# gabinsane/multimodal-vae-comparison

Hardware: AMD Instinct MI355X
Metric: training samples/sec, MoPoE CdSprites+ L2 (fwd+bwd+Adam) (higher is better)
Workload: dtype f32; 1 GPU; configs[1]: MoPoE, CdSprites+ L2 shapes, CNN2 image tower + TxtTransformer text tower, n_latents=32, batch=128/GPU, T=32; Adam(amsgrad) lr 1e-4, beta 1, train mode (dropout on); global_batch=128, parallelism=dp1, settle_steps=40

## Files before the change

### include/mmvae_hip.h

```cpp
#ifndef MMVAE_HIP_H
#define MMVAE_HIP_H

#include <stddef.h>
#include <stdint.h>

#ifdef __cplusplus
extern "C" {
#endif

typedef void* mmvae_stream_t;

enum {
  MMVAE_OK = 0,
  MMVAE_ERR_ARG = 1,
  MMVAE_ERR_UNSUPPORTED = 2,
  MMVAE_ERR_LAUNCH = 3,
  MMVAE_ERR_NO_CONVERGENCE = 4
};

enum { MMVAE_ACT_NONE = 0, MMVAE_ACT_SILU = 1, MMVAE_ACT_RELU = 2, MMVAE_ACT_GELU = 3 };
enum {
  MMVAE_EP_NONE = 0,
  MMVAE_EP_RELU = 1,
  MMVAE_EP_MUL_RELU_MASK = 2,
// ... 26 lines not shown
                                 const mmvae_dropout_t* drop, mmvae_stream_t stream);

int mmvae_ffn32_supported(int d_model, int FF);
int mmvae_proj32_ln_fwd(const float* x, const float* w, const float* b, const float* r, const float* gamma, const float* beta,
                        float* y, float* xhat, float* rstd, int M, const mmvae_dropout_t* drop, mmvae_stream_t stream);
int mmvae_ffn32_bwd_parts(int M, int FF);
size_t mmvae_ffn32_bwd_rowlen(int FF);
int mmvae_ffn32_fwd(const float* x, const float* w1, const float* b1, const float* w2, const float* b2, float* y, int M,
                    int FF, const mmvae_dropout_t* drop, mmvae_stream_t stream);
int mmvae_ffn32_bwd(const float* x, const float* dy, const float* w1, const float* b1, const float* w2, float* dx,
                    float* ws, int M, int FF, const mmvae_dropout_t* drop, mmvae_stream_t stream);
size_t mmvae_ffn32_wsplit_bytes(int FF);
size_t mmvae_ffn32_rsplit_bytes(int M);
int mmvae_ffn32_prep_weights(const float* w1, const float* w2, void* wsplit, int FF, mmvae_stream_t stream);
int mmvae_ffn32_prep_weights_many(const float* const* w1, const float* const* w2, void* const* wsplit, int n, int FF,
                                  mmvae_stream_t stream);
int mmvae_ffn32_fwd_b16(const float* x, const void* wsplit, const float* b1, const float* b2, float* y, int M, int FF,
                        const mmvae_dropout_t* drop, mmvae_stream_t stream);
int mmvae_ffn32_fwd_b16_ln(const float* x, const void* wsplit, const float* b1, const float* b2, const float* r,
                           const float* gamma, const float* beta, float* y, float* xhat, float* rstd, int M, int FF,
                           const mmvae_dropout_t* drop, const mmvae_dropout_t* ln_drop, mmvae_stream_t stream);
int mmvae_ffn32_bwd_b16(const float* x, const float* dy, const void* wsplit, const float* b1, float* dx, float* ws,
                        void* rsplit, const float* dx_add, int M, int FF, const mmvae_dropout_t* drop,
                        mmvae_stream_t stream);

int mmvae_version(void);
const char* mmvae_arch(void);


int mmvae_conv2d_k4s2_fwd(const float* x, const float* w, const float* bias, const float* aux, float* y,
                          int B, int Cin, int Cout, int Hin, int in_act, int ep_mode, mmvae_stream_t stream);

int mmvae_conv2d_k4s2_dgrad(const float* dy, const float* w, const float* aux, float* dx,
                            int B, int Cin, int Cout, int Hout, int ep_mode, mmvae_stream_t stream);

int mmvae_conv2d_k4s2_wgrad(const float* dy, const float* x, float* dw, float* db, float* ws,
                            int B, int Cin, int Cout, int Hout, int x_act, int accumulate, mmvae_stream_t stream);

int mmvae_convT2d_k4s2_fwd(const float* x, const float* w, const float* bias, const float* aux, float* y,
                           int B, int Cin, int Cout, int Hin, int in_act, int ep_mode, mmvae_stream_t stream);

int mmvae_convT2d_k4s2_dgrad(const float* dy, const float* w, const float* aux, float* dx,
                             int B, int Cin, int Cout, int Hin, int ep_mode, mmvae_stream_t stream);

int mmvae_convT2d_k4s2_wgrad(const float* x, const float* dy, float* dw, float* db, float* ws,
                             int B, int Cin, int Cout, int Hin, int x_act, int accumulate, mmvae_stream_t stream);

size_t mmvae_conv_wgrad_ws_floats(int B, int Csmall, int Clarge, int Hsmall);

int mmvae_conv2d_k4s2_bwd(const float* dy, const float* x, const float* w, float* dx, float* dw, float* db, float* ws,
                          int B, int Cin, int Cout, int Hout, int x_act, int accumulate, mmvae_stream_t stream);
int mmvae_convT2d_k4s2_bwd(const float* dy, const float* x, const float* w, float* dx, float* dw, float* db, float* ws,
                           int B, int Cin, int Cout, int Hin, int x_act, int accumulate, mmvae_stream_t stream);
int mmvae_convT3_bce_seeded(const float* x, const float* w, const float* bias, const float* target, float* row,
                            float* dlogit, float* part, unsigned* ticket, int B, int in_act, float seed,
                            mmvae_stream_t stream);
int mmvae_convT3_bce_strips(int B);
int mmvae_conv_plan(int split_bf16);

int mmvae_gemm_f32(const float* A, const float* Bm, const float* bias, const float* aux, float* C,
                   float* a_rowsum, float* ws, int M, int N, int K, long sam, long sak, long sbk, long sbn,
                   long ldc, int a_act, int b_act, int ep_mode, int accumulate, int splitk,
                   mmvae_stream_t stream);
size_t mmvae_gemm_ws_floats(int M, int N, int splitk);
int mmvae_gemm_splits(int M, int N, int K, int splitk);
int mmvae_gemm_b16_set(int on);
int mmvae_bias_group_add(float* y, const float* bias, int rows, int C, int G, mmvae_stream_t stream);
size_t mmvae_bias_group_ws_floats(int rows, int C);
int mmvae_bias_group_parts(int rows);
int mmvae_bias_group_grad(const float* dy, float* db, float* ws, int rows, int C, int G, int accumulate,
                          mmvae_stream_t stream);

int mmvae_linear_fwd(const float* x, const float* w, const float* b, float* aux, float* y, int M, int N, int K,
                     long ldx, int x_act, int ep_mode, mmvae_stream_t stream);
int mmvae_linear_bwd_data(const float* dy, const float* w, const float* aux, float* dx, int M, int N, int K,
                          int ep_mode, int accumulate, mmvae_stream_t stream);
int mmvae_linear_bwd_weight(const float* dy, const float* x, float* dw, float* db, float* ws, int M, int N, int K,
                            long ldx, int x_act, int accumulate, mmvae_stream_t stream);
size_t mmvae_linear_bwd_weight_ws_floats(int M, int N, int K);
#define MMVAE_WGRAD_BATCH_MAX 8
typedef struct {
  const float* dy; const float* x; float* dw; float* db; float* ws;
  int M, N, K; long ldx; int x_act, accumulate;
} mmvae_wgrad_job_t;
int mmvae_linear_bwd_weight_batch(const mmvae_wgrad_job_t* jobs, int n_jobs, mmvae_stream_t stream);
typedef struct {
  const float* dy; const float* x; float* ws;
  int M, N, K;
} mmvae_txt_wgrad_job_t;
int mmvae_txt_wgrad(const mmvae_txt_wgrad_job_t* jobs, int n_jobs, mmvae_stream_t stream);
int mmvae_txt_wgrad_splits(int M, int N, int K);
size_t mmvae_txt_wgrad_ws_floats(int M, int N, int K);
int mmvae_txt_wgrad_supported(int M, int N, int K);
int mmvae_linear_bwd(const float* dy, const float* x, const float* w, const float* aux, float* dx, float* dw,
                     float* db, float* ws, int M, int N, int K, long ldx, int x_act, int ep_mode, int accumulate,
                     mmvae_stream_t stream);
size_t mmvae_linear_bwd_ws_floats(int M, int N, int K);

int mmvae_head_softmax_fwd(float* h, int B, int D, mmvae_stream_t stream);
int mmvae_head_softmax_bwd(const float* h, float* dh, int B, int D, mmvae_stream_t stream);

#define MMVAE_MAX_EXPERTS 8
typedef struct {
  const float* mu[MMVAE_MAX_EXPERTS];
  const float* lv[MMVAE_MAX_EXPERTS];
  const float* eps[MMVAE_MAX_EXPERTS];
// ... 605 lines not shown
```

### multimodal_vae_comparison_amd/csrc/conv.hip

```cpp
#include "conv_common.hpp"

#include "conv_gather.inc"
#include "conv_gather_b16.inc"
#include "conv_scatter.inc"
#include "conv_scatter_b16.inc"
#include "conv_wgrad.inc"

constexpr int cmax(int a, int b) { return a > b ? a : b; }

template <typename G, typename W, bool SPEC = false>
__global__ __launch_bounds__(256) void conv2d_bwd_fused_kernel(ConvScatterArgs ad, ConvWgradArgs aw, int n_w, int w_gx) {
  MMVAE_TRACE_STAMP(10 + G::LGH);
  __shared__ __attribute__((aligned(16))) float smem[cmax(G::SMEM, W::SMEM)];
  if ((int)blockIdx.x < n_w) conv_wgrad_body<W, SPEC>(aw, blockIdx.x % w_gx, blockIdx.x / w_gx, w_gx, smem);
  else
    conv_scatter_body<G>(ad, (n_w & 7) ? (int)blockIdx.x - n_w : xcd_contiguous(blockIdx.x - n_w, gridDim.x - n_w), smem);
}
template <typename G, typename W, bool SPEC = false>
__global__ __launch_bounds__(256) void convT_bwd_fused_kernel(ConvGatherArgs ad, ConvWgradArgs aw, int n_w, int w_gx) {
  MMVAE_TRACE_STAMP(14 - G::LGH);
  __shared__ __attribute__((aligned(16))) float smem[cmax(G::SMEM, W::SMEM)];
  if ((int)blockIdx.x < n_w) conv_wgrad_body<W, SPEC>(aw, blockIdx.x % w_gx, blockIdx.x / w_gx, w_gx, smem);
  else
    conv_gather_body<G, G::RWONLY>(ad, (n_w & 7) ? (int)blockIdx.x - n_w : xcd_contiguous(blockIdx.x - n_w, gridDim.x - n_w),
// ... 175 lines not shown
  if (rc) return rc;
  return conv_bwd_reduce(ws, dw, db, B, Cout, Hin, Cout, accumulate, stream);
}

extern "C" int mmvae_conv2d_k4s2_fwd(const float* x, const float* w, const float* bias, const float* aux, float* y,
                                     int B, int Cin, int Cout, int Hin, int in_act, int ep_mode,
                                     mmvae_stream_t stream) {
  MMVAE_CHECK_ARG(x && w && y && B > 0);
  return conv_gather_dispatch(x, w, bias, aux, y, B, Cin, Cout, Hin, in_act, ep_mode, (hipStream_t)stream);
}
extern "C" int mmvae_conv2d_k4s2_dgrad(const float* dy, const float* w, const float* aux, float* dx, int B, int Cin,
                                       int Cout, int Hout, int ep_mode, mmvae_stream_t stream) {
  MMVAE_CHECK_ARG(dy && w && dx && B > 0);
  return conv_scatter_dispatch(dy, w, nullptr, aux, dx, B, Cout, Cin, Hout, MMVAE_ACT_NONE, ep_mode,
                               (hipStream_t)stream);
}
extern "C" int mmvae_conv2d_k4s2_wgrad(const float* dy, const float* x, float* dw, float* db, float* ws, int B,
                                       int Cin, int Cout, int Hout, int x_act, int accumulate,
                                       mmvae_stream_t stream) {
  MMVAE_CHECK_ARG(dy && x && dw && B > 0);
  return conv_wgrad_dispatch(dy, x, dw, db, ws, B, Cout, Cin, Hout, MMVAE_ACT_NONE, x_act, 1, accumulate,
                             (hipStream_t)stream);
}
extern "C" int mmvae_convT2d_k4s2_fwd(const float* x, const float* w, const float* bias, const float* aux, float* y,
                                      int B, int Cin, int Cout, int Hin, int in_act, int ep_mode,
                                      mmvae_stream_t stream) {
  MMVAE_CHECK_ARG(x && w && y && B > 0);
  return conv_scatter_dispatch(x, w, bias, aux, y, B, Cin, Cout, Hin, in_act, ep_mode, (hipStream_t)stream);
}
extern "C" int mmvae_convT3_bce_seeded(const float* x, const float* w, const float* bias, const float* target, float* row,
                                       float* dlogit, float* part, unsigned* ticket, int B, int in_act, float seed,
                                       mmvae_stream_t stream) {
  MMVAE_CHECK_ARG(x && w && target && row && dlogit && B > 0);
  MMVAE_CHECK_ARG(in_act == MMVAE_ACT_NONE || in_act == MMVAE_ACT_RELU || in_act == MMVAE_ACT_SILU);
  MMVAE_CHECK_ARG(convT3_strips(B) == 1 || (part && ticket));
  MMVAE_CHECK_ARG((((uintptr_t)target | (uintptr_t)dlogit) & 15) == 0);
  ConvT3Args t{x, w, bias, dlogit, target, row, part, ticket, B, in_act, MMVAE_EP_SIGMOID_CLAMP, seed};
  convT3_launch<true>(t, (hipStream_t)stream);
  return mmvae_launch_status();
}
extern "C" int mmvae_convT2d_k4s2_dgrad(const float* dy, const float* w, const float* aux, float* dx, int B, int Cin,
                                        int Cout, int Hin, int ep_mode, mmvae_stream_t stream) {
  MMVAE_CHECK_ARG(dy && w && dx && B > 0);
  return conv_gather_dispatch(dy, w, nullptr, aux, dx, B, Cout, Cin, 2 * Hin, MMVAE_ACT_NONE, ep_mode,
                              (hipStream_t)stream);
}
extern "C" int mmvae_convT2d_k4s2_wgrad(const float* x, const float* dy, float* dw, float* db, float* ws, int B,
                                        int Cin, int Cout, int Hin, int x_act, int accumulate,
                                        mmvae_stream_t stream) {
  MMVAE_CHECK_ARG(x && dy && dw && B > 0);
  return conv_wgrad_dispatch(x, dy, dw, db, ws, B, Cin, Cout, Hin, x_act, MMVAE_ACT_NONE, 2, accumulate,
                             (hipStream_t)stream);
}
extern "C" size_t mmvae_conv_wgrad_ws_floats(int B, int Csmall, int Clarge, int Hsmall) {
  return conv_wgrad_ws_floats(B, Csmall, Clarge, Hsmall);
}
extern "C" int mmvae_conv_wgrad_layout(int B, int Csmall, int Clarge, int Hsmall, int* rows, int* rowlen,
                                       int* bias_col) {
  MMVAE_CHECK_ARG(rows && rowlen && bias_col);
  conv_wgrad_layout(B, Csmall, Clarge, Hsmall, rows, rowlen, bias_col);
  return MMVAE_OK;
}

MMVAE_TRACE_SETTER(conv)

extern "C" int mmvae_conv_plan(int split_bf16) {
  const int old = g_conv_split_bf16;
  if (split_bf16 >= 0) g_conv_split_bf16 = split_bf16 ? 1 : 0;
  return old;
}
```

### multimodal_vae_comparison_amd/hipops.py

```python
import ctypes
import os

import torch

_HERE = os.path.dirname(os.path.abspath(__file__))
LIB_PATH = os.path.join(_HERE, "libmmvae_hip.so")
_lib = None

c_p = ctypes.c_void_p
c_i = ctypes.c_int
c_l = ctypes.c_long
c_f = ctypes.c_float
c_u = ctypes.c_uint
c_sz = ctypes.c_size_t
c_d = ctypes.c_double

MAX_EXPERTS = 8

ACT_NONE, ACT_SILU, ACT_RELU, ACT_GELU = 0, 1, 2, 3
EP_NONE, EP_RELU, EP_MUL_RELU_MASK, EP_MUL_SILU_GRAD, EP_GELU, EP_MUL_GELU_GRAD, EP_SIGMOID_CLAMP, EP_SIGMOID, EP_ADD_AUX = range(9)

ERR_ARG, ERR_UNSUPPORTED, ERR_LAUNCH, ERR_NO_CONVERGENCE = 1, 2, 3, 4
_ERR = {ERR_ARG: "invalid argument", ERR_UNSUPPORTED: "unsupported shape", ERR_LAUNCH: "kernel launch failed",
        ERR_NO_CONVERGENCE: "no convergence within the iteration cap"}
# ... 64 lines not shown

class RcStat(ctypes.Structure):
    _fields_ = [("Y", c_p), ("mean", c_p), ("rstd", c_p), ("gamma", c_p), ("pqr", c_p), ("dgamma", c_p), ("dbeta", c_p),
                ("part", c_p), ("counter", c_p), ("acc", c_i), ("eval", c_i)]


class RcGeom(ctypes.Structure):
    _fields_ = [("H", c_i), ("W", c_i), ("Ho", c_i), ("Wo", c_i), ("KW", c_i), ("S", c_i), ("P", c_i)]


class RcFwd(ctypes.Structure):
    _fields_ = [("x", c_p), ("w", c_p), ("xmean", c_p), ("xsc", c_p), ("xbeta", c_p), ("y", c_p), ("ws", c_p),
                ("tile_ticket", c_p), ("M", c_i), ("Cin", c_i), ("Cout", c_i), ("T", c_i), ("pre", c_i), ("g", RcGeom),
                ("gamma", c_p),
                ("beta", c_p), ("run_mean", c_p), ("run_var", c_p), ("mean", c_p), ("rstd", c_p), ("sc", c_p), ("part", c_p),
                ("counter", c_p), ("eps", c_f), ("momentum", c_f), ("eval", c_i)]


class RcDgrad(ctypes.Structure):
    _fields_ = [("G", c_p), ("Y", c_p), ("pqr", c_p), ("w", c_p), ("add", c_p), ("add_tbl", c_p), ("mask", c_i),
                ("mY", c_p), ("mmean", c_p), ("msc", c_p), ("mbeta", c_p), ("out", c_p), ("ws", c_p), ("tile_ticket", c_p),
                ("row_map", c_p), ("M", c_i), ("Min", c_i), ("Cin", c_i), ("Cout", c_i), ("T", c_i), ("nstat", c_i), ("g", RcGeom),
                ("st", RcStat * 2)]


class RcWgrad(ctypes.Structure):
    _fields_ = [("G", c_p), ("Y", c_p), ("pqr", c_p), ("x", c_p), ("xmean", c_p), ("xsc", c_p), ("xbeta", c_p), ("tbl", c_p),
                ("dw", c_p), ("ws", c_p), ("counter", c_p), ("M", c_i), ("Cin", c_i), ("Cout", c_i), ("T", c_i), ("pre", c_i),
                ("accumulate", c_i)]


RC_MAX_JOBS = 8


class RcJob(ctypes.Structure):
    _fields_ = [("kind", c_i), ("f", RcFwd), ("d", RcDgrad), ("w", RcWgrad)]


c_dp = ctypes.POINTER(Dropout)
DROPOUT_SLOTS = 16

SIGNATURES = {
    "mmvae_version": (c_i, []),
    "mmvae_arch": (ctypes.c_char_p, []),
    "mmvae_conv2d_k4s2_fwd": (c_i, [c_p] * 5 + [c_i] * 6 + [c_p]),
    "mmvae_conv2d_k4s2_dgrad": (c_i, [c_p] * 4 + [c_i] * 5 + [c_p]),
    "mmvae_conv2d_k4s2_wgrad": (c_i, [c_p] * 5 + [c_i] * 6 + [c_p]),
    "mmvae_convT2d_k4s2_fwd": (c_i, [c_p] * 5 + [c_i] * 6 + [c_p]),
    "mmvae_convT2d_k4s2_dgrad": (c_i, [c_p] * 4 + [c_i] * 5 + [c_p]),
    "mmvae_convT2d_k4s2_wgrad": (c_i, [c_p] * 5 + [c_i] * 6 + [c_p]),
    "mmvae_conv_wgrad_ws_floats": (c_sz, [c_i] * 4),
    "mmvae_conv2d_k4s2_bwd": (c_i, [c_p] * 7 + [c_i] * 6 + [c_p]),
    "mmvae_convT2d_k4s2_bwd": (c_i, [c_p] * 7 + [c_i] * 6 + [c_p]),
    "mmvae_gemm_f32": (c_i, [c_p] * 7 + [c_i] * 3 + [c_l] * 5 + [c_i] * 5 + [c_p]),
    "mmvae_gemm_ws_floats": (c_sz, [c_i] * 3),
    "mmvae_gemm_splits": (c_i, [c_i] * 4),
    "mmvae_bias_group_add": (c_i, [c_p, c_p, c_i, c_i, c_i, c_p]),
    "mmvae_bias_group_grad": (c_i, [c_p, c_p, c_p, c_i, c_i, c_i, c_i, c_p]),
    "mmvae_bias_group_ws_floats": (c_sz, [c_i, c_i]),
    "mmvae_bias_group_parts": (c_i, [c_i]),
    "mmvae_linear_fwd": (c_i, [c_p] * 5 + [c_i] * 3 + [c_l] + [c_i] * 2 + [c_p]),
    "mmvae_gemm_b16_set": (c_i, [c_i]),
    "mmvae_attn_t_bwd_set": (c_i, [c_i]),
    "mmvae_attn_path": (c_i, [c_i] * 4 + [c_l] * 3 + [c_i]),
    "mmvae_linear_bwd_data": (c_i, [c_p] * 4 + [c_i] * 5 + [c_p]),
    "mmvae_linear_bwd_weight": (c_i, [c_p] * 5 + [c_i] * 3 + [c_l] + [c_i] * 2 + [c_p]),
    "mmvae_linear_bwd_weight_ws_floats": (c_sz, [c_i] * 3),
    "mmvae_linear_bwd_weight_batch": (c_i, [c_p, c_i, c_p]),
    "mmvae_txt_layer_plan": (c_i, [c_i] * 3),
    "mmvae_conv_plan": (c_i, [c_i]),
    "mmvae_convT3_bce_seeded": (c_i, [c_p] * 8 + [c_i, c_i, c_f, c_p]),
    "mmvae_convT3_bce_strips": (c_i, [c_i]),
    "mmvae_txt_wgrad": (c_i, [c_p, c_i, c_p]),
    "mmvae_txt_wgrad_splits": (c_i, [c_i] * 3),
    "mmvae_txt_wgrad_ws_floats": (c_sz, [c_i] * 3),
    "mmvae_txt_wgrad_supported": (c_i, [c_i] * 3),
    "mmvae_input_pipe_create": (c_i, [c_p, c_p, c_sz]),
    "mmvae_input_pipe_destroy": (c_i, [c_p]),
    "mmvae_input_pipe_prefetch": (c_i, [c_p, c_p]),
    "mmvae_input_pipe_commit": (c_i, [c_p, c_p, c_i, c_p, c_p]),
    "mmvae_linear_bwd": (c_i, [c_p] * 8 + [c_i] * 3 + [c_l] + [c_i] * 3 + [c_p]),
    "mmvae_linear_bwd_ws_floats": (c_sz, [c_i] * 3),
    "mmvae_head_softmax_fwd": (c_i, [c_p, c_i, c_i, c_p]),
    "mmvae_head_softmax_bwd": (c_i, [c_p, c_p, c_i, c_i, c_p]),
    "mmvae_poe_reparam_kl_fwd": (c_i, [ctypes.POINTER(PoeFwdArgs), c_p, c_p, c_p, c_i, c_i, c_i, c_u, c_i, c_i, c_i,
                                       c_i, c_p, c_p]),
    "mmvae_poe_reparam_kl_bwd": (c_i, [ctypes.POINTER(PoeBwdArgs), c_p, c_p, c_p, c_p, c_p, c_i, c_i, c_i, c_u, c_i, c_i,
                                       c_i, c_i, c_i, c_p]),
    "mmvae_poe_reparam_kl_bwd_acc": (c_i, [ctypes.POINTER(PoeBwdArgs), c_p, c_p, c_p, c_p, c_p, c_i, c_i, c_i, c_u, c_i,
                                           c_i, c_i, c_i, c_i, c_u, c_p]),
    "mmvae_poe_ws_floats": (c_sz, [c_i, c_i]),
    "mmvae_bce_rowsum_fwd": (c_i, [c_p] * 3 + [c_i] * 3 + [c_p]),
    "mmvae_bce_sigmoid_clamp_bwd": (c_i, [c_p] * 4 + [c_i] * 3 + [c_p]),
    "mmvae_bce_rowsum_bwd": (c_i, [c_p] * 4 + [c_i] * 2 + [c_p]),
    "mmvae_sigmoid_clamp_bwd": (c_i, [c_p] * 3 + [c_l] + [c_p]),
    "mmvae_bce_elem_fwd": (c_i, [c_p] * 3 + [c_l] + [c_p]),
    "mmvae_bce_rowsum_seeded": (c_i, [c_p] * 3 + [c_f] + [c_p] + [c_i] * 2 + [c_p]),
    "mmvae_ce_over_time_seeded": (c_i, [c_p] * 3 + [c_f] + [c_p] + [c_i] * 3 + [c_p]),
    "mmvae_lprob_elem_fwd": (c_i, [c_p] * 3 + [c_l, c_l, c_f, c_i, c_p]),
    "mmvae_lprob_elem_bwd": (c_i, [c_p] * 4 + [c_l, c_l, c_f, c_i, c_p]),
    "mmvae_optimal_sigma_elem_fwd": (c_i, [c_p] * 5 + [c_l, c_p]),
    "mmvae_optimal_sigma_elem_bwd": (c_i, [c_p] * 6 + [c_l, c_p]),
    "mmvae_pointwise_rowsum_fwd": (c_i, [c_p] * 3 + [c_i] * 4 + [c_p]),
    "mmvae_pointwise_rowsum_bwd": (c_i, [c_p] * 4 + [c_i] * 4 + [c_p]),
    "mmvae_pointwise_elem": (c_i, [c_p] * 4 + [c_l, c_i, c_p]),
    "mmvae_ce_over_time_fwd": (c_i, [c_p] * 4 + [c_i] * 4 + [c_p]),
# ... 159 lines not shown
    "mmvae_rc_stem_wgrad_ws_floats": (c_sz, [c_i] * 4),
    "mmvae_rc_stem_wgrad": (c_i, [c_p] * 8 + [c_i] * 4 + [ctypes.POINTER(RcGeom), c_i, c_p]),
    "mmvae_rc_wgrad_splits": (c_i, [c_i] * 4),
    "mmvae_rc_wgrad_ws_floats": (c_sz, [c_i] * 4),
    "mmvae_rc_wgrad_tickets": (c_sz, [c_i] * 3),
    "mmvae_rc_blockout": (c_i, [c_p] * 8 + [c_i, c_p, c_l, c_i, c_p]),
    "mmvae_rc_bn_apply": (c_i, [c_p] * 5 + [c_l, c_i, c_p]),
    "mmvae_dropout_advance": (c_i, [c_p, c_u, c_p]),
    "mmvae_dropout_advance_many": (c_i, [c_p, c_i, c_p]),
    "mmvae_dropout_mask": (c_i, [c_dp, c_p, c_l, c_p]),
    "mmvae_dropout_act_fwd": (c_i, [c_p, c_p, c_l, c_i, c_dp, c_p]),
    "mmvae_dropout_act_bwd": (c_i, [c_p, c_p, c_p, c_l, c_i, c_dp, c_p]),
    "mmvae_head_bcast_dropout_fwd": (c_i, [c_p, c_p] + [c_i] * 4 + [c_dp, c_p]),
    "mmvae_head_bcast_dropout_bwd": (c_i, [c_p, c_p] + [c_i] * 4 + [c_dp, c_p]),
    "mmvae_conv_wgrad_layout": (c_i, [c_i] * 4 + [c_p] * 3),
    "mmvae_linear_bwd_weight_splits": (c_i, [c_i] * 3),
    "mmvae_linear_bwd_splits": (c_i, [c_i] * 3),
    "mmvae_layernorm_bwd_rows": (c_i, [c_i, c_i]),
    "mmvae_embed_bwd_rows": (c_i, [c_i] * 3),
}
ACC_DEFER = 2
MAX_SEGMENTS = 64


LC_MAX_ROWS, LC_MAX_OUT = 32, 4


class RowPtrs(ctypes.Structure):
    _fields_ = [("p", c_p * LC_MAX_ROWS)]


class GPtrs(ctypes.Structure):
    _fields_ = [("g", c_p * LC_MAX_OUT)]


INPUT_MAX_MODS = 8
INPUT_IMAGE_U8, INPUT_TEXT_TOKENS = 0, 1


class InputMod(ctypes.Structure):
    _fields_ = [("kind", c_i), ("src_off", c_sz), ("len_off", c_sz), ("dst", c_p), ("mask", c_p), ("n", c_l),
                ("B", c_i), ("T", c_i), ("V", c_i)]


WGRAD_BATCH_MAX = 8
DROPOUT_ADVANCE_MAX = 16


class WgradJob(ctypes.Structure):
    _fields_ = [("dy", c_p), ("x", c_p), ("dw", c_p), ("db", c_p), ("ws", c_p), ("M", c_i), ("N", c_i), ("K", c_i),
                ("ldx", c_l), ("x_act", c_i), ("accumulate", c_i)]


class TxtWgradJob(ctypes.Structure):
    _fields_ = [("dy", c_p), ("x", c_p), ("ws", c_p), ("M", c_i), ("N", c_i), ("K", c_i)]


TXT_WGRAD_MAX = 8


class TxtLayerW(ctypes.Structure):
    _fields_ = [(k, c_p) for k in ("in_w", "in_b", "out_w", "out_b", "l1_w", "l1_b", "l2_w", "l2_b", "n1_g", "n1_b",
                                   "n2_g", "n2_b", "n3_g", "n3_b", "x_in_w", "x_in_b", "x_out_w", "x_out_b")]


class TxtLayerSaved(ctypes.Structure):
    _fields_ = [(k, c_p) for k in ("qkv", "probs", "ao", "xhat1", "rstd1", "x1", "vproj", "vb", "xhat2", "rstd2", "x2",
                                   "h1", "g", "xhatf", "rstdf")]


class TxtLayerGrads(ctypes.Structure):
    _fields_ = [(k, c_p) for k in ("d_f", "d_h1", "d_ca", "d_v", "d_a", "d_qkv", "lnws")]


class TxtLayerDrop(ctypes.Structure):
    _fields_ = [(k, Dropout) for k in ("attn", "drop1", "xattn", "drop2", "ffn", "drop3")]


class ReduceSegments(ctypes.Structure):
    _fields_ = [("src", c_p * MAX_SEGMENTS), ("dst", c_p * MAX_SEGMENTS), ("rows", c_i * MAX_SEGMENTS),
                ("len", c_i * MAX_SEGMENTS), ("stride", c_i * MAX_SEGMENTS), ("blk0", c_i * MAX_SEGMENTS),
                ("next", c_i * MAX_SEGMENTS), ("n", c_i)]


def lib():
    global _lib
    if _lib is None:
        if not os.path.exists(LIB_PATH):
            raise RuntimeError(
                f"{LIB_PATH} is missing: build it with __graft_entry__.build() or "
                f"`make -C multimodal_vae_comparison_amd/csrc` (hipcc --offload-arch=gfx950). There is no fallback path.")
        L = ctypes.CDLL(os.environ.get("MMVAE_HIP_LIB", LIB_PATH))
        for name, (res, args) in SIGNATURES.items():
            fn = getattr(L, name)
            fn.restype = res
            fn.argtypes = args
        _lib = L
    return _lib


def check(rc, name):
    if rc != 0:
        raise RuntimeError(f"{name} failed: {_ERR.get(rc, rc)}")


def stream():
# ... 37 lines not shown
```

### multimodal_vae_comparison_amd/models/mmvae_models.py

```python
import os
from itertools import chain, combinations

import torch
import torch.distributions as dist

from .. import ops
from .mmvae_base import TorchMMVAE, normal, packed_head
from .objectives import recon_rowsum


def _uses(t, stream):
    if t is not None and t.is_cuda and stream is not None:
        base = t._base if t._base is not None else t
        base.record_stream(stream)


class MoPOE(TorchMMVAE):

    def __init__(self, vaes, n_latents: int, obj_config: dict, model_config=None):
        super().__init__(vaes, n_latents, **obj_config)
        self.model_config = model_config
        self.modelName = "mopoe"
        self._require_normal_priors()
        self.subsets = self.set_subsets()
# ... 19 lines not shown
        self._begin_step()
        names = list(self.vaes.keys())
        M = len(names)
        dev = next(v["data"] for v in mods.values() if v["data"] is not None).device
        main_tower = 0
        streams = self._tower_streams(dev, main_tower)
        cur = torch.cuda.current_stream(dev)
        real = [cur if st is None else st for st in streams]
        self._fork(streams, dev, mods)
        B, D = next(v["data"] for v in mods.values() if v["data"] is not None).shape[0], self.n_latents
        W = self._elbo_weights(B)
        eps_mode = "fused"
        if self.eps_override is not None and eps_mode == "fused":
            eps_mode = "after"
        eps = self._draw_many(M, B, D, dev) if eps_mode == "first" else None
        enc = [None] * M
        enc_order = list(enumerate(zip(names, streams)))
        for i, (n, st) in enc_order:
            with torch.cuda.stream(st):
                tower = self.vaes[n].enc
                tower.raw_heads = True
                ops.Marks.mark(f"enc {n} start")
                try:
                    mu_lv = tower(mods[n])
                finally:
                    tower.raw_heads = False
                enc[i] = tuple(ops.mark_tensor(t, f"enc {n} out[{j}]") for j, t in enumerate(mu_lv))
                if eps is None and i == 0 and eps_mode == "after":
                    eps = self._draw_many(M, B, D, dev)
        rotate = True
        fuse = real[-1] if rotate else real[0]
        self._fuse_stream = fuse0 = fuse
        for st in real:
            if st != fuse:
                fuse.wait_stream(st)
        theta = self._pz_params[1]
        for t in list(eps or []) + [t for pair in enc for t in pair]:
            _uses(t, fuse)
        with torch.cuda.stream(fuse):
            packed = [packed_head(mu, lv) for mu, lv in enc]
            if seeds is not None and getattr(self, "early_adam", None) is not None and ops.GradReducer.defer_next:
                packed[-1] = ops.EarlyStepPoint.apply(packed[-1])
            if eps is None:
                _, kl, z = ops.poe_reparam_kl(theta, packed, M, True, (1 << (M + 1)) - 1, theta.grad, raw=True,
                                              rng=self._rng_state)
            else:
                _, kl, z = ops.poe_reparam_kl(theta, packed, eps, True, (1 << (M + 1)) - 1, theta.grad, raw=True)
        _uses(kl, cur)
        for st in real:
            if st != fuse:
                st.wait_stream(fuse)
        recs = [None] * M
        order = [(i, names[i], real[(i + M - 1) % M] if rotate else real[i]) for i in range(M)]
        for i, n, st in order:
            vae = self.vaes[n]
            _uses(z[i], st)
            with torch.cuda.stream(st):
                zi = ops.mark_tensor(z[i], f"dec {n} z")
                if seeds is not None and getattr(self, "early_adam", None) is not None and ops.GradReducer.defer_next:
                    zi = ops.DecoderEnd.apply(zi)
                if seeds is not None and st != fuse0 and ops.GradReducer.side_head is not None:
                    zi = ops.StreamIdlePoint.apply(zi)
                if seeds is not None:
                    with ops.ConstSeed(seeds[i], W[0][i]):
                        fuse = vae.ltype == "bce" and mods[n]["masks"] is None
                        out, _ = vae.dec({"latents": zi.unsqueeze(0), "masks": mods[n]["masks"],
                                          "bce_target": mods[n]["data"] if fuse else None})
                        r = recon_rowsum(vae.ltype, out, mods[n], laplace=self._lap(vae))
                else:
                    out, _ = vae.dec({"latents": zi.unsqueeze(0), "masks": mods[n]["masks"]})
                    r = recon_rowsum(vae.ltype, out, mods[n], laplace=self._lap(vae))
                recs[i] = ops.mark_tensor(r, f"dec {n} recon")
            _uses(recs[i], cur)
        self._fusion_inputs = packed
        return recs, kl, W, streams, dev

    def objective(self, mods):
        recs, kl, W, streams, dev = self._elbo_terms(mods)
        self._join(streams, dev)
        ops.Marks.mark("joined decoders")
        out = ops.lincomb_rows(recs + [kl], W)
        return {"loss": out[0], "kld": out[1], "reconstruction_loss": recs}

    def backward_encoders(self):
        hs, dhs, streams, dev = self._cut
        self._cut = None
        for st in streams:
            if st is not None:
                ops.GradReducer.note_stream(dev, st)
        torch.autograd.backward(hs, list(dhs))
        self._join(streams, dev)

    def objective_backward(self, mods, cut=False):
        first = next(v["data"] for v in mods.values() if v["data"] is not None)
        B, dev, M = first.shape[0], first.device, len(self.vaes)
        W = self._elbo_weights(B)
        key = (tuple(W[0]), B, str(dev))
        if getattr(self, "_seed_key", None) != key:
            self._seeds = [torch.full((B,), W[0][i], device=dev) for i in range(M)]
            self._seeds.append(torch.tensor(W[0][M:], device=dev).reshape(-1, 1).expand(M + 1, B).contiguous())
            self._seed_key = key
        recs, kl, W, streams, dev = self._elbo_terms(mods, self._seeds)
        def assemble(stream):
            with torch.cuda.stream(stream), torch.no_grad():
                return ops.lincomb_rows([r.detach() for r in recs] + [kl.detach()], W)

        out = None
        tail = ops.GradReducer.tail = ops.lincomb_rows_args(recs + [kl], W)
        early = getattr(self, "early_adam", None)
        if early is not None and not cut and ops.GradReducer.defer_next:
            ops.GradReducer.early_step = (early[0], self._fuse_stream, early[1], early[2])
            ops.GradReducer.dw_open = True
        if cut:
            self._cut = (list(self._fusion_inputs), torch.autograd.grad(recs + [kl], self._fusion_inputs, self._seeds),
                         streams, dev)
        else:
            torch.autograd.backward(recs + [kl], self._seeds)
        ops.GradReducer.tail = ops.GradReducer.early_step = None
        ops.GradReducer.dw_open = ops.GradReducer.early_ready = False
        if tail is not None and tail["done"]:
            out = tail["args"][2].unbind(0)
        if out is None:
            self._join(streams, dev)
            out = assemble(None)
        self._unjoined = (streams, dev)
        return {"loss": out[0], "kld": out[1], "reconstruction_loss": recs}

    def finish_step(self):
        pending, self._unjoined = getattr(self, "_unjoined", None), None
        if pending is not None:
            self._join(*pending)

    def modality_mixing(self, input_batch):
        latents = {}
        enc_mods = self.encode(input_batch)
        latents["modalities"] = enc_mods
        distr_subsets, last = {}, None
        n_all = len(self.vaes)
        for s_key, mods in self.subsets.items():
            if all(m.modelName in input_batch and input_batch[m.modelName]["data"] is not None for m in mods):
                mus = [enc_mods[m.modelName]["shared"][0] for m in mods]
                lvs = [enc_mods[m.modelName]["shared"][1] for m in mods]
                s_mu, s_var = self.product_of_experts(mus, lvs, with_prior=(len(mods) == n_all))
                distr_subsets[s_key] = [s_mu.unsqueeze(0), s_var.unsqueeze(0)]
                last = (s_mu, s_var)
        self.weights = (1 / float(len(distr_subsets))) * torch.ones(len(distr_subsets), device=last[0].device)
        latents["joint"] = [last[0], last[1]]
        latents["subsets"] = distr_subsets
        return latents

    def _proposal_size(self, n_given):
        return 2 ** n_given - 1

    def _proposal(self, mods, given):
        subsets = self.modality_mixing(self._given_only(mods, given))["subsets"]
        comps = torch.stack([torch.cat([mu[0], var[0]], -1) for mu, var in subsets.values()])
        return comps, [False] * comps.shape[0]

    def _sample(self, x, K=1, of=None):
        latents = self.modality_mixing(x)
        j_mu, j_var = latents["joint"]
        return latents, ((mod, j_mu + j_var * self._draws(K, *j_mu.shape, j_mu.device)) for mod in self.vaes)

    def _unimodal(self, head):
        return {m: (*q["shared"], dist.Normal) for m, q in head["modalities"].items() if q["shared"] is not None}

    def forward(self, inputs, K=1):
        latents, zs = self._sample(inputs, K)
        qz_d, px_d, z_d, qz_joint = {}, {}, {}, {}
        for mod, z in zs:
            vae = self.vaes[mod]
            sh = latents["modalities"][mod]["shared"]
# ... 573 lines not shown
```

### multimodal_vae_comparison_amd/ops.py

```python
import bisect
import ctypes
import itertools
import math
import os

import numpy as np
import torch
from torch.autograd import Function

from . import hipops as H

_DACT = {H.ACT_NONE: H.EP_NONE, H.ACT_SILU: H.EP_MUL_SILU_GRAD, H.ACT_RELU: H.EP_MUL_RELU_MASK,
         H.ACT_GELU: H.EP_MUL_GELU_GRAD}


CALLS = [0]


def _call(name, *args):
    CALLS[0] += 1
    H.check(getattr(H.lib(), name)(*args), name)


class GradReducer:

    enabled = True
    tail = None
    defer_next = False
    deferred = None
    pre_join = None
    side_tail = None
    side_head = None
    _arena = {}
    _state = {}

    @classmethod
    def _st(cls, device):
        key = H.device_key(device)
        st = cls._state.get(key)
        if st is None:
            st = {"off": 0, "segs": [], "armed": False, "device": device, "keep": [], "used": set(), "spill": [],
                  "spilled": 0}
            cls._state[key] = st
        return key, st

    @classmethod
    def begin_step(cls, device):
        if device.type != "cuda":
            return
        _, st = cls._st(device)
        cls.early_step, cls.dw_jobs, cls.dw_open = None, [], False
        cls.tw_jobs, cls.early_ready = {}, False
        cls.last_writer.clear()
        cls.packed_grads.clear()
        cls.packed_uses.clear()
        if cls.deferred is not None:
            cls.deferred = None
            raise RuntimeError("GradReducer: a deferred fold was never taken by an optimiser step: the split weight "
                               "gradients of the previous backward pass were lost")
        if st["armed"] or st["segs"]:
            st.update(off=0, segs=[], armed=False, keep=[], used=set(), spill=[], spilled=0)
            cls.tail = None

    @classmethod
    def alloc(cls, n_floats, device):
        key, st = cls._st(device)
        n = (int(n_floats) + 63) // 64 * 64
        ar = cls._arena.get(key)
        if ar is None or st["off"] + n > ar.numel():
            if ar is not None:
                st["spill"].append(ar)
                st["spilled"] += ar.numel()
            ar = torch.empty(max(n, 16 << 20), dtype=torch.float32, device=device)
            cls._arena[key] = ar
            st["off"] = 0
            if device.type == "cuda" and StreamPlan.enabled:
                cur = torch.cuda.current_stream(device)
                for other in set(StreamPlan.pair.get(key, ())) | set(st["used"]):
                    if other != cur:
                        other.wait_stream(cur)
        out = ar[st["off"]:st["off"] + n]
        st["off"] += n
        return out

    @classmethod
    def add(cls, src_ptr, dst, rows, length, stride):
        _, st = cls._st(dst.device)
        st["segs"].append((src_ptr, dst.data_ptr(), int(rows), int(length), int(stride)))
        if not st["armed"]:
            st["armed"] = True
            dev = dst.device
            torch.autograd.Variable._execution_engine.queue_callback(lambda: cls.flush(dev))

    @classmethod
    def _merged(cls, segs):
        if not cls.merge_adjacent or len(segs) < 2:
            return list(segs)
        runs = []
        for sp, dp, r, ln, sd in segs:
            if runs:
                q = runs[-1]
                tot = sum(q[4])
                if sp == q[0] + 4 * tot and dp == q[1] + 4 * tot and r == q[2] and sd == q[3]:
                    q[4].append(ln)
                    continue
# ... 42 lines not shown
    packed_grads, packed_uses = {}, {}
    share_packed_grads = True

    @classmethod
    def packed_grads_done(cls):
        left = [k for k, (_, n) in cls.packed_grads.items() if n > 0]
        for k in cls.packed_grads:
            cls.packed_uses.pop(k, None)
        cls.packed_grads.clear()
        if left:
            raise RuntimeError(f"PoeReparamKL: {len(left)} head output(s) were read by more column-range fusion calls than "
                               f"took part in this backward pass; their gradient was not delivered "
                               f"(ops.GradReducer.share_packed_grads = False restores one gradient tensor per call)")
    merge_adjacent = True

    dw_jobs = []
    dw_open = False
    dw_later_enabled = os.environ.get("MMVAE_LINEAR_DW_LATER", "1") == "1"

    last_writer = {}

    @classmethod
    def writes(cls, device, *grads):
        if device.type != "cuda":
            return
        cur = torch.cuda.current_stream(device)
        for g in grads:
            if g is None:
                continue
            k = g.data_ptr()
            last = cls.last_writer.get(k)
            if last is not None and last != cur:
                cur.wait_stream(last)
            cls.last_writer[k] = cur

    @classmethod
    def dw_later(cls, device):
        es = cls.early_step
        return (cls.dw_later_enabled and cls.dw_open and es is not None and torch.cuda.current_stream(device) == es[1]
                and len(cls.dw_jobs) < H.WGRAD_BATCH_MAX)

    @classmethod
    def flush_dw(cls):
        jobs, cls.dw_jobs = cls.dw_jobs, []
        if not jobs:
            return
        arr = (H.WgradJob * len(jobs))()
        cls.writes(jobs[0][0].device, *[t for job in jobs for t in job[2:4]])
        for j, (dy, x, dw, db, M, N, K, x_act) in zip(arr, jobs):
            j.dy, j.x, j.dw, j.db, j.ws = H.ptr(dy), H.ptr(x), H.ptr(dw), H.ptr(db), None
            j.M, j.N, j.K, j.ldx, j.x_act, j.accumulate = M, N, K, K, x_act, H.ACC_DEFER
        _call("mmvae_linear_bwd_weight_batch", ctypes.cast(arr, ctypes.c_void_p), len(jobs), H.stream())

    tw_jobs = {}
    tw_enabled = os.environ.get("MMVAE_SKINNY_DW", "1") == "1"
    TW_MIN_ROWS, TW_MAX_N, TW_MAX_K = 2048, 162, 128

    @classmethod
    def tw_ok(cls, M, N, K, in_act, has_b, dy, x):
        return (cls.tw_enabled and M >= cls.TW_MIN_ROWS and N <= cls.TW_MAX_N and K <= cls.TW_MAX_K and in_act == H.ACT_NONE
                and has_b and TXT_WGRAD and dy.is_contiguous() and x.is_contiguous()
                and H.lib().mmvae_txt_wgrad_supported(M, N, K))

    @classmethod
    def tw_park(cls, job):
        dev = job[0].device
        st = torch.cuda.current_stream(dev)
        lst = cls.tw_jobs.setdefault(st, [])
        lst.append(job)
        cls.note_stream(dev, st)
        cls.ensure_flush(dev)
        if len(lst) >= H.TXT_WGRAD_MAX:
            cls.tw_jobs[st] = []
            _txt_wgrad(lst)

    @classmethod
    def tw_flush_stream(cls, st):
        lst = cls.tw_jobs.pop(st, None)
        if lst:
            _txt_wgrad(lst)

    @classmethod
    def tw_flush(cls):
        jobs, cls.tw_jobs = cls.tw_jobs, {}
        for st, lst in jobs.items():
            if lst:
                with torch.cuda.stream(st):
                    _txt_wgrad(lst)

    @classmethod
    def run_early_step(cls, device):
        es = cls.early_step
        if es is None or not cls.early_ready:
            return
        fn, stream, lo, hi = es
        _, st = cls._st(device)
        if torch.cuda.current_stream(device) != stream:
            return
        cls.early_step = None
        if st["spill"] or not cls.defer_next:
            return
        inside = cls._merged([sg for sg in st["segs"] if lo <= sg[1] < hi])
        if len(inside) > H.MAX_SEGMENTS or any(sg[1] + 4 * sg[3] > hi for sg in inside):
            return
        st["segs"] = [sg for sg in st["segs"] if not (lo <= sg[1] < hi)]
        fn(cls._table(inside) if inside else None)

    @classmethod
    def keep(cls, device, *tensors):
        cls._st(device)[1]["keep"].extend(t for t in tensors if t is not None)

    @classmethod
    def note_stream(cls, device, stream):
        cls._st(device)[1]["used"].add(stream)

    @classmethod
    def ensure_flush(cls, device):
        _, st = cls._st(device)
        if not st["armed"]:
            st["armed"] = True
            torch.autograd.Variable._execution_engine.queue_callback(lambda: cls.flush(device))

    @classmethod
    def flush(cls, device):
        cls.flush_dw()
        cls.tw_flush()
        _, st = cls._st(device)
        cur = torch.cuda.current_stream(device)
        if cls.pre_join is not None:
            cls.pre_join(device, [s_ for s_ in st["used"] if s_ != cur])
        for side in st["used"]:
            if side != cur:
                cur.wait_stream(side)
        st["used"] = set()
        st["keep"] = []
        segs, st["segs"], st["armed"] = cls._merged(st["segs"]), [], False
        cls._check_disjoint(segs)
        need, st["off"] = st["spilled"] + st["off"], 0
        tail, cls.tail = cls.tail, None
        defer, cls.defer_next = cls.defer_next, False
        if defer and 0 < len(segs) <= H.MAX_SEGMENTS and not st["spill"]:
            cls.deferred = {"table": cls._table(segs), "tail": tail, "device": device}
            if tail is not None:
                tail["done"] = True
            return
        for i in range(0, len(segs), H.MAX_SEGMENTS):
            t = cls._table(segs[i:i + H.MAX_SEGMENTS])
            if tail is not None and i + H.MAX_SEGMENTS >= len(segs):
                rp, flat, out, n, B, k = tail["args"]
                _call("mmvae_reduce_segments_lincomb", ctypes.byref(t), ctypes.byref(rp), flat, H.ptr(out), n, B, k,
                      H.stream())
                tail["done"] = True
            else:
                _call("mmvae_reduce_segments", ctypes.byref(t), H.stream())
        if st["spill"]:
            st["spill"], st["spilled"] = [], 0
            if not torch.cuda.is_current_stream_capturing():
                cls._arena[H.device_key(device)] = torch.empty(need + (1 << 20), dtype=torch.float32, device=device)


class Marks:
    enabled = os.environ.get("MMVAE_MARKS", "0") == "1"
    names = []
    buf = None

    @classmethod
    def mark(cls, name):
        if not cls.enabled:
            return
        if cls.buf is None:
            cls.buf = torch.zeros(256, dtype=torch.int64, device="cuda")
        if name not in cls.names:
            cls.names.append(name)
        i = cls.names.index(name)
        _call("mmvae_debug_timestamp", cls.buf.data_ptr() + 8 * i, H.stream())


class Mark(Function):
# ... 136 lines not shown
                  B, Cin, Cout, Hout, in_act, acc, H.stream())
        else:
            _call("mmvae_conv2d_k4s2_wgrad", H.ptr(dy), H.ptr(x), H.ptr(dw), H.ptr(db), H.ptr(ws), B, Cin, Cout, Hout,
                  in_act, acc, H.stream())
        if defer:
            _conv_segments(ws, dw, db, B, Cout, Cin, Hout, Cout)
        return dx, ret_w, ret_b, None, None, None


class ConvT2dK4S2(Function):

    @staticmethod
    def forward(ctx, x, w, b, in_act, out_ep, gw, gb, ep_bwd=True):
        x = H.f32c(x)
        B, Cin, Hin, _ = x.shape
        Cout = w.shape[1]
        y = torch.empty(B, Cout, 2 * Hin, 2 * Hin, device=x.device, dtype=torch.float32)
        _call("mmvae_convT2d_k4s2_fwd", H.ptr(x), H.ptr(w), H.ptr(b), None, H.ptr(y), B, Cin, Cout, Hin, in_act,
              out_ep, H.stream())
        if not ep_bwd:
            out_ep = H.EP_NONE
        ctx.save_for_backward(x, w, y if out_ep in (H.EP_SIGMOID_CLAMP, H.EP_SIGMOID) else None)
        ctx.cfg = (in_act, out_ep, gw, gb, b is not None)
        return y

    @staticmethod
    def backward(ctx, dy):
        x, w, y = ctx.saved_tensors
        in_act, out_ep, gw, gb, has_b = ctx.cfg
        dy = H.f32c(dy)
        B, Cin, Hin, _ = x.shape
        Cout = w.shape[1]
        if out_ep == H.EP_SIGMOID_CLAMP:
            dl = torch.empty_like(dy)
            _call("mmvae_sigmoid_clamp_bwd", H.ptr(dy), H.ptr(y), H.ptr(dl), dy.numel(), H.stream())
            dy = dl
        elif out_ep == H.EP_SIGMOID:
            dl = torch.empty_like(dy)
            _call("mmvae_sigmoid_bwd", H.ptr(dy), H.ptr(y), H.ptr(dl), dy.numel(), H.stream())
            dy = dl
        dx, ret_w, ret_b = _convT_k4s2_bwd(x, w, dy, in_act, gw, gb, has_b, ctx.needs_input_grad[0])
        return dx, ret_w, ret_b, None, None, None, None, None


def _convT_k4s2_bwd(x, w, dy, in_act, gw, gb, has_b, need_dx):
    B, Cin, Hin, _ = x.shape
    Cout = w.shape[1]
    dw, db, acc_w, ret_w, ret_b = _grad_dst(w, gw, gb, has_b, Cout)
    nws = H.lib().mmvae_conv_wgrad_ws_floats(B, Cin, Cout, Hin)
    defer = _defer(gw, gb if has_b else gw)
    ws = GradReducer.alloc(nws, x.device) if defer else H.workspace(nws, x.device)
    acc = H.ACC_DEFER if defer else acc_w
    dx = None
    if need_dx:
        dx = torch.empty_like(x)
        _call("mmvae_convT2d_k4s2_bwd", H.ptr(dy), H.ptr(x), H.ptr(w), H.ptr(dx), H.ptr(dw), H.ptr(db), H.ptr(ws),
              B, Cin, Cout, Hin, in_act, acc, H.stream())
    else:
        _call("mmvae_convT2d_k4s2_wgrad", H.ptr(x), H.ptr(dy), H.ptr(dw), H.ptr(db), H.ptr(ws), B, Cin, Cout, Hin,
              in_act, acc, H.stream())
    if defer:
        _conv_segments(ws, dw, db, B, Cin, Cout, Hin, Cout)
    return dx, ret_w, ret_b


_T3_SCRATCH = {}


class ConvT3Bce(Function):

    calls = 0

    @staticmethod
    def forward(ctx, x, w, b, in_act, gw, gb, target, cs):
        ConvT3Bce.calls += 1
        x, target = H.f32c(x), H.f32c(target)
        B = x.shape[0]
        dev = x.device
        row = torch.empty(B, device=dev)
        dl = torch.empty(B, 3, 64, 64, device=dev)
        S = H.lib().mmvae_convT3_bce_strips(B)
        part = tick = None
        if S > 1:
            key = (dev.index, H.stream(), B)
            ent = _T3_SCRATCH.get(key)
            if ent is None:
                assert not torch.cuda.is_current_stream_capturing(), \
                    "ConvT3Bce: first call at this batch size inside a graph capture (run one eager warm-up step first)"
                ent = _T3_SCRATCH[key] = (torch.zeros(B * S, device=dev), torch.zeros(B, dtype=torch.int32, device=dev))
            part, tick = ent
        _call("mmvae_convT3_bce_seeded", H.ptr(x), H.ptr(w), H.ptr(b), H.ptr(target), H.ptr(row), H.ptr(dl), H.ptr(part),
              H.ptr(tick), B, in_act, cs.value, H.stream())
        ctx.save_for_backward(x, w, dl)
        ctx.cfg = (in_act, gw, gb, b is not None, cs.seed.data_ptr(), cs.value)
        return row

    @staticmethod
    def backward(ctx, g):
        x, w, dl = ctx.saved_tensors
        in_act, gw, gb, has_b, seed_ptr, seed_value = ctx.cfg
        if g.data_ptr() != seed_ptr:
            dl = dl * (H.f32c(g) / seed_value).view(-1, 1, 1, 1)
        dx, ret_w, ret_b = _convT_k4s2_bwd(x, w, dl, in_act, gw, gb, has_b, ctx.needs_input_grad[0])
        return dx, ret_w, ret_b, None, None, None, None, None


CONVT3_BCE = True
# ... 589 lines not shown
                t.g[s_][j], t.ld[s_][j] = g.data_ptr() + 4 * (r * B * W + c0), W
                t.n_g[s_] = j + 1
        t.n, t.B = n, B
        if n:
            _call("mmvae_rows_fan_bwd", ctypes.byref(t), H.stream())
        return (None, *outs)


def rows_fan(plan, srcs):
    return list(RowsFan.apply(plan, *srcs))


class KlRow(Function):

    @staticmethod
    def forward(ctx, kl, j):
        ctx.shape, ctx.j = tuple(kl.shape), int(j)
        return kl[int(j)]

    @staticmethod
    def backward(ctx, g):
        out = torch.empty(ctx.shape, device=g.device, dtype=g.dtype)
        out[ctx.j].copy_(g)
        return out, None


def kl_row(kl, j):
    return KlRow.apply(kl, j)


class DecoderEnd(Function):

    @staticmethod
    def forward(ctx, z):
        return z.view_as(z)

    @staticmethod
    def backward(ctx, g):
        GradReducer.tw_flush_stream(torch.cuda.current_stream(g.device))
        return g


class EarlyStepPoint(Function):

    @staticmethod
    def forward(ctx, x):
        return x.view_as(x)

    @staticmethod
    def backward(ctx, g):
        GradReducer.early_ready = True
        GradReducer.dw_open = False
        GradReducer.flush_dw()
        return g


class StreamIdlePoint(Function):

    @staticmethod
    def forward(ctx, z):
        return z.view_as(z)

    @staticmethod
    def backward(ctx, g):
        fn, GradReducer.side_head = GradReducer.side_head, None
        if fn is not None:
            fn(g.device)
        return g


def poe_reparam_kl(theta, packed, eps, with_prior, kl_mask, gtheta=None, cols=None, raw=False, rng=None):
    assert not (raw and cols is not None), "raw heads: the softmax runs over the full head width"
    assert not (raw and int(with_prior) == 2), "raw heads: the pass-through posterior (with_prior = 2) takes lv as its scale"
    if rng is not None:
        out = PoeReparamKL.apply(theta, gtheta, with_prior, int(eps), kl_mask, len(packed), cols, raw, rng, *packed)
    else:
        out = PoeReparamKL.apply(theta, gtheta, with_prior, len(eps), kl_mask, len(packed), cols, raw, None, *packed,
                                 *eps)
    return out[0], out[1], list(out[2:])


class BceRowsum(Function):

    @staticmethod
    def forward(ctx, x_hat, target):
        x_hat, target = H.f32c(x_hat), H.f32c(target)
        B = x_hat.shape[0]
        F = x_hat.numel() // B
        row = torch.empty(B, device=x_hat.device)
        _call("mmvae_bce_rowsum_fwd", H.ptr(x_hat), H.ptr(target), H.ptr(row), B, F, B, H.stream())
        ctx.save_for_backward(x_hat, target)
        return row

    @staticmethod
    def backward(ctx, g):
        x_hat, target = ctx.saved_tensors
        B = x_hat.shape[0]
        F = x_hat.numel() // B
        dx = torch.empty_like(x_hat)
        _call("mmvae_bce_rowsum_bwd", H.ptr(x_hat), H.ptr(target), H.ptr(H.f32c(g)), H.ptr(dx), B, F, H.stream())
        return dx, None


class BceElem(Function):

    @staticmethod
# ... 2810 lines not shown
```

Baseline: 333,500 samples/s.

## Defer convT weight-grad jobs and batch them on an idle side stream

For the image decoder's transposed convolutions, backward now runs only the dgrad kernel inline on the fusion stream. The weight-gradient work is parked and later launched as one batched wgrad kernel covering up to four layers, on the other modality's idle stream. An event makes the early optimizer step wait for it. The aim is to take wgrad off the critical path, overlap it with the other tower's backward, and save launches, at the cost of more cross-stream sync and tighter stream-lifetime bookkeeping.

```diff
diff --git a/include/mmvae_hip.h b/include/mmvae_hip.h
--- a/include/mmvae_hip.h
+++ b/include/mmvae_hip.h
@@ -102,6 +102,12 @@
                           int B, int Cin, int Cout, int Hout, int x_act, int accumulate, mmvae_stream_t stream);
 int mmvae_convT2d_k4s2_bwd(const float* dy, const float* x, const float* w, float* dx, float* dw, float* db, float* ws,
                            int B, int Cin, int Cout, int Hin, int x_act, int accumulate, mmvae_stream_t stream);
+#define MMVAE_CONV_WGRAD_BATCH_MAX 4
+typedef struct {
+  const float* x; const float* dy; float* ws;
+  int B, Cin, Cout, Hin, x_act, has_bias;
+} mmvae_conv_wgrad_job_t;
+int mmvae_conv_wgrad_batch(const mmvae_conv_wgrad_job_t* jobs, int n_jobs, mmvae_stream_t stream);
 int mmvae_convT3_bce_seeded(const float* x, const float* w, const float* bias, const float* target, float* row,
                             float* dlogit, float* part, unsigned* ticket, int B, int in_act, float seed,
                             mmvae_stream_t stream);
diff --git a/multimodal_vae_comparison_amd/csrc/conv.hip b/multimodal_vae_comparison_amd/csrc/conv.hip
--- a/multimodal_vae_comparison_amd/csrc/conv.hip
+++ b/multimodal_vae_comparison_amd/csrc/conv.hip
@@ -251,6 +251,70 @@
   return conv_wgrad_dispatch(x, dy, dw, db, ws, B, Cin, Cout, Hin, x_act, MMVAE_ACT_NONE, 2, accumulate,
                              (hipStream_t)stream);
 }
+struct ConvWgradBatch {
+  ConvWgradArgs a[MMVAE_CONV_WGRAD_BATCH_MAX];
+  int blk0[MMVAE_CONV_WGRAD_BATCH_MAX + 1];
+  int gx[MMVAE_CONV_WGRAD_BATCH_MAX];
+  int q3[MMVAE_CONV_WGRAD_BATCH_MAX];
+  int n;
+};
+template <typename W32, bool SPEC>
+__global__ __launch_bounds__(256) void conv_wgrad_batch_kernel(ConvWgradBatch bt) {
+  MMVAE_TRACE_STAMP(40);
+  using W3 = WgradGeom<3, 5>;
+  __shared__ __attribute__((aligned(16))) float smem[cmax(W3::SMEM, W32::SMEM)];
+  int p = 0;
+#pragma unroll
+  for (int q = 1; q < MMVAE_CONV_WGRAD_BATCH_MAX; ++q) p = (q < bt.n && (int)blockIdx.x >= bt.blk0[q]) ? q : p;
+  const int local = blockIdx.x - bt.blk0[p], gx = bt.gx[p];
+  if (bt.q3[p]) conv_wgrad_body<W3, SPEC>(bt.a[p], local % gx, local / gx, gx, smem);
+  else conv_wgrad_body<W32, SPEC>(bt.a[p], local % gx, local / gx, gx, smem);
+}
+
+extern "C" int mmvae_conv_wgrad_batch(const mmvae_conv_wgrad_job_t* jobs, int n_jobs, mmvae_stream_t stream) {
+  MMVAE_CHECK_ARG(jobs && n_jobs >= 1);
+  if (n_jobs > MMVAE_CONV_WGRAD_BATCH_MAX) return MMVAE_ERR_UNSUPPORTED;
+  ConvWgradBatch bt;
+  bt.n = n_jobs;
+  bt.blk0[0] = 0;
+  int spec = -1, qc8 = -1;
+  for (int p = 0; p < n_jobs; ++p) {
+    const mmvae_conv_wgrad_job_t& j = jobs[p];
+    MMVAE_CHECK_ARG(j.x && j.dy && j.ws && j.B > 0);
+    const bool l3 = j.Cin == 32 && j.Cout == 3 && j.Hin == 32, l32 = j.Cin == 32 && j.Cout == 32 && j.Hin == 16;
+    if (!(l3 || l32) || j.x_act == MMVAE_ACT_GELU) return MMVAE_ERR_UNSUPPORTED;
+    const int n_macro = wgrad_n_macro(j.B, j.Hin), nsplit = wgrad_splits(n_macro, j.Cout);
+    const int s = wgrad_spec(n_macro, nsplit) ? 1 : 0;
+    if (spec >= 0 && s != spec) return MMVAE_ERR_UNSUPPORTED;
+    spec = s;
+    int nch = 1;
+    if (l32) {
+      const int c8 = wgrad_qc8(nsplit, n_macro) ? 1 : 0;
+      if (qc8 >= 0 && c8 != qc8) return MMVAE_ERR_UNSUPPORTED;
+      qc8 = c8;
+      nch = c8 ? WgradGeom<32, 4, 8>::NCH : WgradGeom<32, 4>::NCH;
+    }
+    bt.a[p] = ConvWgradArgs{j.x, j.dy, j.ws, j.B, j.x_act, MMVAE_ACT_NONE, j.has_bias ? 2 : 0, n_macro, 32,
+                            (long)32 * j.Cout * 16 + 32};
+    bt.gx[p] = nsplit;
+    bt.q3[p] = l3 ? 1 : 0;
+    bt.blk0[p + 1] = bt.blk0[p] + nsplit * nch;
+  }
+  for (int p = n_jobs; p < MMVAE_CONV_WGRAD_BATCH_MAX; ++p) {
+    bt.a[p] = bt.a[0]; bt.gx[p] = 1; bt.q3[p] = 0; bt.blk0[p + 1] = bt.blk0[n_jobs];
+  }
+  const dim3 grid(bt.blk0[n_jobs]);
+  hipStream_t st = (hipStream_t)stream;
+  if (qc8 != 0) {
+    if (spec) hipLaunchKernelGGL((conv_wgrad_batch_kernel<WgradGeom<32, 4, 8>, true>), grid, dim3(256), 0, st, bt);
+    else hipLaunchKernelGGL((conv_wgrad_batch_kernel<WgradGeom<32, 4, 8>, false>), grid, dim3(256), 0, st, bt);
+  } else {
+    if (spec) hipLaunchKernelGGL((conv_wgrad_batch_kernel<WgradGeom<32, 4>, true>), grid, dim3(256), 0, st, bt);
+    else hipLaunchKernelGGL((conv_wgrad_batch_kernel<WgradGeom<32, 4>, false>), grid, dim3(256), 0, st, bt);
+  }
+  return mmvae_launch_status();
+}
+
 extern "C" size_t mmvae_conv_wgrad_ws_floats(int B, int Csmall, int Clarge, int Hsmall) {
   return conv_wgrad_ws_floats(B, Csmall, Clarge, Hsmall);
 }
diff --git a/multimodal_vae_comparison_amd/hipops.py b/multimodal_vae_comparison_amd/hipops.py
--- a/multimodal_vae_comparison_amd/hipops.py
+++ b/multimodal_vae_comparison_amd/hipops.py
@@ -140,6 +140,7 @@
     "mmvae_conv_wgrad_ws_floats": (c_sz, [c_i] * 4),
     "mmvae_conv2d_k4s2_bwd": (c_i, [c_p] * 7 + [c_i] * 6 + [c_p]),
     "mmvae_convT2d_k4s2_bwd": (c_i, [c_p] * 7 + [c_i] * 6 + [c_p]),
+    "mmvae_conv_wgrad_batch": (c_i, [c_p, c_i, c_p]),
     "mmvae_gemm_f32": (c_i, [c_p] * 7 + [c_i] * 3 + [c_l] * 5 + [c_i] * 5 + [c_p]),
     "mmvae_gemm_ws_floats": (c_sz, [c_i] * 3),
     "mmvae_gemm_splits": (c_i, [c_i] * 4),
@@ -405,6 +406,14 @@
                 ("ldx", c_l), ("x_act", c_i), ("accumulate", c_i)]
 
 
+CONV_WGRAD_BATCH_MAX = 4
+
+
+class ConvWgradJob(ctypes.Structure):
+    _fields_ = [("x", c_p), ("dy", c_p), ("ws", c_p), ("B", c_i), ("Cin", c_i), ("Cout", c_i), ("Hin", c_i),
+                ("x_act", c_i), ("has_bias", c_i)]
+
+
 class TxtWgradJob(ctypes.Structure):
     _fields_ = [("dy", c_p), ("x", c_p), ("ws", c_p), ("M", c_i), ("N", c_i), ("K", c_i)]
 
diff --git a/multimodal_vae_comparison_amd/models/mmvae_models.py b/multimodal_vae_comparison_amd/models/mmvae_models.py
--- a/multimodal_vae_comparison_amd/models/mmvae_models.py
+++ b/multimodal_vae_comparison_amd/models/mmvae_models.py
@@ -95,6 +95,7 @@
                 st.wait_stream(fuse)
         recs = [None] * M
         order = [(i, names[i], real[(i + M - 1) % M] if rotate else real[i]) for i in range(M)]
+        self._idle_stream = next((st for _, _, st in reversed(order) if st != fuse0), None)
         for i, n, st in order:
             vae = self.vaes[n]
             _uses(z[i], st)
@@ -154,6 +155,8 @@
         if early is not None and not cut and ops.GradReducer.defer_next:
             ops.GradReducer.early_step = (early[0], self._fuse_stream, early[1], early[2])
             ops.GradReducer.dw_open = True
+        if not cut and ops.GradReducer.defer_next and self._idle_stream is not None and M == 2:
+            ops.GradReducer.cw_streams = (self._fuse_stream, self._idle_stream)
         if cut:
             self._cut = (list(self._fusion_inputs), torch.autograd.grad(recs + [kl], self._fusion_inputs, self._seeds),
                          streams, dev)
@@ -161,6 +164,7 @@
             torch.autograd.backward(recs + [kl], self._seeds)
         ops.GradReducer.tail = ops.GradReducer.early_step = None
         ops.GradReducer.dw_open = ops.GradReducer.early_ready = False
+        ops.GradReducer.cw_streams = None
         if tail is not None and tail["done"]:
             out = tail["args"][2].unbind(0)
         if out is None:
diff --git a/multimodal_vae_comparison_amd/ops.py b/multimodal_vae_comparison_amd/ops.py
--- a/multimodal_vae_comparison_amd/ops.py
+++ b/multimodal_vae_comparison_amd/ops.py
@@ -51,6 +51,7 @@
         _, st = cls._st(device)
         cls.early_step, cls.dw_jobs, cls.dw_open = None, [], False
         cls.tw_jobs, cls.early_ready = {}, False
+        cls.cw_jobs, cls.cw_done, cls.cw_streams = [], None, None
         cls.last_writer.clear()
         cls.packed_grads.clear()
         cls.packed_uses.clear()
@@ -199,6 +200,51 @@
             j.M, j.N, j.K, j.ldx, j.x_act, j.accumulate = M, N, K, K, x_act, H.ACC_DEFER
         _call("mmvae_linear_bwd_weight_batch", ctypes.cast(arr, ctypes.c_void_p), len(jobs), H.stream())
 
+    cw_jobs = []
+    cw_enabled = os.environ.get("MMVAE_CONV_DW_LATER", "1") == "1"
+    CW_MAX_BATCH = {(32, 3, 32): 128, (32, 32, 16): 64}
+    cw_streams = None
+    cw_done = None
+
+    @classmethod
+    def cw_later(cls, device, shape):
+        st = cls.cw_streams
+        return (cls.cw_enabled and st is not None and torch.cuda.current_stream(device) == st[0]
+                and shape[0] <= cls.CW_MAX_BATCH.get(tuple(shape[1:]), 0) and len(cls.cw_jobs) < H.CONV_WGRAD_BATCH_MAX)
+
+    @classmethod
+    def cw_park(cls, job):
+        cls.cw_jobs.append(job)
+        B = job[5][0]
+        if len(cls.cw_jobs) < sum(B <= m for m in cls.CW_MAX_BATCH.values()):
+            return None
+        dev = job[0].device
+        ev = torch.cuda.current_stream(dev).record_event()
+        return lambda: cls._cw_launch(dev, ev)
+
+    @classmethod
+    def _cw_launch(cls, dev, ev):
+        side = cls.cw_streams[1]
+        side.wait_event(ev)
+        for j in cls.cw_jobs:
+            for t in j[:2]:
+                (t._base if t._base is not None else t).record_stream(side)
+        with torch.cuda.stream(side):
+            cls.flush_cw()
+            cls.cw_done = side.record_event()
+        cls.note_stream(dev, side)
+
+    @classmethod
+    def flush_cw(cls):
+        jobs, cls.cw_jobs = cls.cw_jobs, []
+        if not jobs:
+            return
+        arr = (H.ConvWgradJob * len(jobs))()
+        for j, (x, dy, dw, db, ws, (B, Cin, Cout, Hin), x_act) in zip(arr, jobs):
+            j.x, j.dy, j.ws = H.ptr(x), H.ptr(dy), H.ptr(ws)
+            j.B, j.Cin, j.Cout, j.Hin, j.x_act, j.has_bias = B, Cin, Cout, Hin, x_act, int(db is not None)
+        _call("mmvae_conv_wgrad_batch", ctypes.cast(arr, ctypes.c_void_p), len(jobs), H.stream())
+
     tw_jobs = {}
     tw_enabled = os.environ.get("MMVAE_SKINNY_DW", "1") == "1"
     TW_MIN_ROWS, TW_MAX_N, TW_MAX_K = 2048, 162, 128
@@ -251,6 +297,7 @@
         if len(inside) > H.MAX_SEGMENTS or any(sg[1] + 4 * sg[3] > hi for sg in inside):
             return
         st["segs"] = [sg for sg in st["segs"] if not (lo <= sg[1] < hi)]
+        assert cls.cw_done is None
         fn(cls._table(inside) if inside else None)
 
     @classmethod
@@ -271,6 +318,7 @@
     @classmethod
     def flush(cls, device):
         cls.flush_dw()
+        cls.flush_cw()
         cls.tw_flush()
         _, st = cls._st(device)
         cur = torch.cuda.current_stream(device)
@@ -513,7 +561,15 @@
     ws = GradReducer.alloc(nws, x.device) if defer else H.workspace(nws, x.device)
     acc = H.ACC_DEFER if defer else acc_w
     dx = None
-    if need_dx:
+    if need_dx and defer and GradReducer.cw_later(x.device, (B, Cin, Cout, Hin)):
+        dx = torch.empty_like(x)
+        go = GradReducer.cw_park((x, dy, dw, db, ws, (B, Cin, Cout, Hin), in_act))
+        ep = _DACT[in_act]
+        _call("mmvae_convT2d_k4s2_dgrad", H.ptr(dy), H.ptr(w), H.ptr(x) if ep else None, H.ptr(dx), B, Cin, Cout, Hin, ep,
+              H.stream())
+        if go is not None:
+            go()
+    elif need_dx:
         dx = torch.empty_like(x)
         _call("mmvae_convT2d_k4s2_bwd", H.ptr(dy), H.ptr(x), H.ptr(w), H.ptr(dx), H.ptr(dw), H.ptr(db), H.ptr(ws),
               B, Cin, Cout, Hin, in_act, acc, H.stream())
@@ -1209,6 +1265,9 @@
         GradReducer.early_ready = True
         GradReducer.dw_open = False
         GradReducer.flush_dw()
+        done, GradReducer.cw_done = GradReducer.cw_done, None
+        if done is not None:
+            torch.cuda.current_stream(g.device).wait_event(done)
         return g
 
 
```

After: 339,100 samples/s, median of 6. +1.7%, better.
